# Keep-Passion/ImageStitch

Measured on AMD Instinct MI355X. Metric: image-pairs/sec (2048x2048 grayscale, SURF+BF), higher is better.
Workload: dtype f32

## Files before the change

### imagestitch_amd/csrc/match_kernels.hip

```cpp
#include "common.h"
#include <algorithm>
#include <stdlib.h>
#include <math.h>

typedef float float2v __attribute__((ext_vector_type(2)));
typedef const float __attribute__((address_space(4))) cfloat;
typedef float f16v __attribute__((ext_vector_type(16)));

#define SLOAD16(dst, ptr) asm volatile("s_load_dwordx16 %0, %1, 0x0" : "=s"(dst) : "s"(ptr))
#define SLOAD16_BEFORE(dst, ptr, live) asm volatile("s_load_dwordx16 %0, %2, 0x0" : "=s"(dst), "+s"(live) : "s"(ptr))
#define SWAIT(dst) asm volatile("s_waitcnt lgkmcnt(0)" : "+s"(dst))
#define SWAIT2(d0, d1) asm volatile("s_waitcnt lgkmcnt(0)" : "+s"(d0), "+s"(d1))
#define BF_CHUNK(buf, base)                                                                    \
    _Pragma("unroll") for (int d = 0; d < 16; d += 4) {                                        \
        float2v e0 = qv[base + d + 0] - buf[d + 0];                                            \
        float2v e1 = qv[base + d + 1] - buf[d + 1];                                            \
        float2v e2 = qv[base + d + 2] - buf[d + 2];                                            \
        float2v e3 = qv[base + d + 3] - buf[d + 3];                                            \
        acc += e0 * e0 + e1 * e1 + e2 * e2 + e3 * e3;                                          \
    }

__device__ __forceinline__ void knn_update(float dsq, int j, float &b1, float &b2, int &i1, float &b1sq, float &b2sq)
{
    if (dsq < b2sq) {
// ... 204 lines not shown
                S.m1 = fminf(S.m1, v);
                S.thr = S.m2 + BFM_MARGIN;
            }
        }
    }
}

__global__ __launch_bounds__(256, 2) void k_bf_mfma_d64(const MatchDev *jobs)
{
    const MatchDev &J = jobs[blockIdx.z];
    const int nq = __builtin_amdgcn_readfirstlane(*J.nq_ptr), nt = __builtin_amdgcn_readfirstlane(*J.nt_ptr);
    const int lane = threadIdx.x & 63, wave = threadIdx.x >> 6;
    const int q0 = (blockIdx.x * 4 + wave) * 64;
    if (q0 >= nq) return;
    const int nsplit = gridDim.y, sp = blockIdx.y;
    const int ntiles = (nt + 31) >> 5;
    const int tchunk = (ntiles + nsplit - 1) / nsplit;
    const int tile0 = sp * tchunk, tile1 = min(ntiles, tile0 + tchunk);
    const int col = lane & 31, half = lane >> 5;
    float bq0[32], bq1[32];
    {
        const float4 *p0 = reinterpret_cast<const float4 *>(J.q + (size_t)min(q0 + col, nq - 1) * 64 + 32 * half);
        const float4 *p1 = reinterpret_cast<const float4 *>(J.q + (size_t)min(q0 + 32 + col, nq - 1) * 64 + 32 * half);
#pragma unroll
        for (int s4 = 0; s4 < 8; s4++) {
            const float4 u = p0[s4], v = p1[s4];
            bq0[4 * s4 + 0] = -2.f * u.x; bq0[4 * s4 + 1] = -2.f * u.y; bq0[4 * s4 + 2] = -2.f * u.z; bq0[4 * s4 + 3] = -2.f * u.w;
            bq1[4 * s4 + 0] = -2.f * v.x; bq1[4 * s4 + 1] = -2.f * v.y; bq1[4 * s4 + 2] = -2.f * v.z; bq1[4 * s4 + 3] = -2.f * v.w;
        }
    }
    const float baug = half == 0 ? 1.f : 0.f;
    const bool va = q0 + col < nq, vb = q0 + 32 + col < nq;
    BfmState Sa = {INFINITY, INFINITY, INFINITY, 0}, Sb = {INFINITY, INFINITY, INFINITY, 0};
    const size_t pitch = (size_t)J.capq;
    const int lst = sp * 2 + half;
    uint2 *lista = J.c_ent + (size_t)lst * BFM_CAPL * pitch + (q0 + col), *listb = lista + 32;
    const float *T = J.t;
    for (int pass = 0; pass < 2; pass++) {
        const int tend = pass == 0 ? min(tile0 + 1, tile1) : tile1;
        float4 an[8];
        if (tile0 < tend) {
            const float4 *pn = reinterpret_cast<const float4 *>(T + (size_t)min(tile0 * 32 + col, nt - 1) * 64 + 32 * half);
#pragma unroll
            for (int s4 = 0; s4 < 8; s4++) an[s4] = pn[s4];
        }
        for (int tl = tile0; tl < tend; tl++) {
            float a[32];
#pragma unroll
            for (int s4 = 0; s4 < 8; s4++) { a[4 * s4] = an[s4].x; a[4 * s4 + 1] = an[s4].y; a[4 * s4 + 2] = an[s4].z; a[4 * s4 + 3] = an[s4].w; }
            if (tl + 1 < tend) {
                const float4 *pn = reinterpret_cast<const float4 *>(T + (size_t)min((tl + 1) * 32 + col, nt - 1) * 64 + 32 * half);
#pragma unroll
                for (int s4 = 0; s4 < 8; s4++) an[s4] = pn[s4];
            }
            float part = 0.f;
#pragma unroll
            for (int s = 0; s < 32; s++) part += a[s] * a[s];
            const float tnorm = part + __shfl_xor(part, 32, 64);
            const float aaug = half == 0 ? (tl * 32 + col < nt ? tnorm : BFM_FAR) : 0.f;
            f16v acc0 = {0, 0, 0, 0, 0, 0, 0, 0, 0, 0, 0, 0, 0, 0, 0, 0}, acc1 = acc0;
#pragma unroll
            for (int s = 0; s < 32; s++) {
                acc0 = __builtin_amdgcn_mfma_f32_32x32x2f32(a[s], bq0[s], acc0, 0, 0, 0);
                acc1 = __builtin_amdgcn_mfma_f32_32x32x2f32(a[s], bq1[s], acc1, 0, 0, 0);
            }
            acc0 = __builtin_amdgcn_mfma_f32_32x32x2f32(aaug, baug, acc0, 0, 0, 0);
            acc1 = __builtin_amdgcn_mfma_f32_32x32x2f32(aaug, baug, acc1, 0, 0, 0);
            if (pass == 0) {
                bfm_warm(acc0, Sa); bfm_warm(acc1, Sb);
            } else {
                const int row0 = tl * 32 + 4 * half;
                bfm_scan(acc0, Sa, row0, lista, pitch, tl != tile0); bfm_scan(acc1, Sb, row0, listb, pitch, tl != tile0);
            }
        }
        if (pass == 0) {
            Sa.thr = va ? Sa.m2 + BFM_MARGIN : -INFINITY;
            Sb.thr = vb ? Sb.m2 + BFM_MARGIN : -INFINITY;
        }
    }
    if (va) J.c_cnt[(size_t)lst * pitch + q0 + col] = Sa.cnt;
    if (vb) J.c_cnt[(size_t)lst * pitch + q0 + 32 + col] = Sb.cnt;
}

#define BF16_ROW 144
#define BF16_FRAGS 9
typedef short s8v __attribute__((ext_vector_type(8)));

__device__ __forceinline__ unsigned short bf16_rne(float x)
{
    unsigned u = __float_as_uint(x);
    u += 0x7fffu + ((u >> 16) & 1u);
    return (unsigned short)(u >> 16);
}
__device__ __forceinline__ float bf16_to_f32(unsigned short h) { return __uint_as_float((unsigned)h << 16); }

__global__ __launch_bounds__(256) void k_bf_split16(const MatchDev *jobs, float scale_q)
{
    const MatchDev &J = jobs[blockIdx.z];
    const bool is_t = blockIdx.y == 1;
    const int n = is_t ? *J.nt_ptr : *J.nq_ptr;
    const int row = blockIdx.x * 128 + (threadIdx.x >> 1), half = threadIdx.x & 1;
    if (row >= n) return;
    const float *src = (is_t ? J.t : J.q) + (size_t)row * 64 + 32 * half;
    const float sc = is_t ? 1.f : scale_q;
    float part = 0.f;
    s8v hi[4], lo[4];
#pragma unroll
    for (int d = 0; d < 32; d++) {
        const float x = src[d];
        part += x * x;
        const float xs = x * sc;
        const unsigned short h = bf16_rne(xs);
        hi[d >> 3][d & 7] = (short)h;
        lo[d >> 3][d & 7] = (short)bf16_rne(xs - bf16_to_f32(h));
    }
    const float tot = part + __shfl_xor(part, 1, 64);
    s8v ns = {0, 0, 0, 0, 0, 0, 0, 0};
    if (half == 0) {
        unsigned short a = 0x3f80, b = 0x3f80;
        if (is_t) { a = bf16_rne(tot); b = bf16_rne(tot - bf16_to_f32(a)); }
        ns[0] = (short)a; ns[1] = (short)b;
    }
    if (is_t) {
        s8v *dst = reinterpret_cast<s8v *>(J.t16) + (size_t)(row >> 5) * (BF16_FRAGS * 64) + (row & 31) + 32 * half;
#pragma unroll
        for (int s4 = 0; s4 < 4; s4++) { dst[s4 * 64] = hi[s4]; dst[(4 + s4) * 64] = lo[s4]; }
        dst[8 * 64] = ns;
    } else {
        s8v *dst = reinterpret_cast<s8v *>(J.q16 + (size_t)row * BF16_ROW + 64 * half);
#pragma unroll
        for (int s4 = 0; s4 < 4; s4++) { dst[s4] = hi[s4]; dst[4 + s4] = lo[s4]; }
        if (half == 0) *reinterpret_cast<s8v *>(J.q16 + (size_t)row * BF16_ROW + 128) = ns;
    }
}

#ifndef VFSMS_BF_SKIP
#define VFSMS_BF_SKIP 0
#endif
#ifndef BFM_GLDS
#define BFM_GLDS 1
#endif
#define BFM_HI_ERR 1.6e-2f
#define GASM __attribute__((address_space(1)))
typedef GASM const s8v *g_cs8v;
typedef float f2v __attribute__((ext_vector_type(2)));

#ifdef VFSMS_DESC_TIMING
__device__ unsigned long long g_bf_cycles[2][8];
extern "C" int vfsms_debug_bf_cycles(unsigned long long *out) { return hipMemcpyFromSymbol(out, HIP_SYMBOL(g_bf_cycles), sizeof(unsigned long long) * 16) == hipSuccess ? 0 : -3; }
#define BT_DECL unsigned long long _bt[5] = {0, 0, 0, 0, 0}, _bt0 = clock64(), _btl = _bt0
#define BT_MARK(ph) do { const unsigned long long _n = clock64(); _bt[ph] += _n - _btl; _btl = _n; } while (0)
#define BT_FLUSH(pass) do { if ((threadIdx.x & 63) == 0) { for (int _q = 0; _q < 5; _q++) atomicAdd(&g_bf_cycles[pass][_q], _bt[_q]); \
        atomicAdd(&g_bf_cycles[pass][5], clock64() - _bt0); atomicAdd(&g_bf_cycles[pass][6], 1ull); } } while (0)
#else
#define BT_DECL do {} while (0)
#define BT_MARK(ph) do {} while (0)
#define BT_FLUSH(pass) do {} while (0)
#endif
template <int PASS>
__global__ __launch_bounds__(256, 3) void k_bf_mfma16_d64(const MatchDev *jobs, int qblocks, int nsplit, int njobs)
{
    unsigned unit, qb;
    xcd_roi_map(blockIdx.x, (unsigned)qblocks, (unsigned)(nsplit * njobs), unit, qb);
    const int sp = (int)(unit % (unsigned)nsplit);
    const MatchDev &J = jobs[unit / (unsigned)nsplit];
    const int nq = __builtin_amdgcn_readfirstlane(*J.nq_ptr), nt = __builtin_amdgcn_readfirstlane(*J.nt_ptr);
    const int lane = threadIdx.x & 63, wave = threadIdx.x >> 6;
    if ((int)qb * 256 >= nq) return;
    BT_DECL;
    const int q0 = ((int)qb * 4 + wave) * 64;
    const bool live = q0 < nq;
    const int ntiles = (nt + 31) >> 5;
    const int tchunk = (ntiles + nsplit - 1) / nsplit;
    const int tile0 = sp * tchunk, tile1 = min(ntiles, tile0 + tchunk);
    const int col = lane & 31, half = lane >> 5;
    const s8v zero = {0, 0, 0, 0, 0, 0, 0, 0};
    s8v bh0[4], bl0[4], bh1[4], bl1[4], bn0, bn1;
    {
        g_cs8v p0 = (g_cs8v)(J.q16 + (size_t)min(q0 + col, nq - 1) * BF16_ROW + 64 * half);
        g_cs8v p1 = (g_cs8v)(J.q16 + (size_t)min(q0 + 32 + col, nq - 1) * BF16_ROW + 64 * half);
#pragma unroll
        for (int s4 = 0; s4 < 4; s4++) {
            bh0[s4] = p0[s4]; bh1[s4] = p1[s4];
            if (PASS == 1) { bl0[s4] = p0[4 + s4]; bl1[s4] = p1[4 + s4]; } else { bl0[s4] = zero; bl1[s4] = zero; }
        }
        bn0 = half == 0 ? *(g_cs8v)(J.q16 + (size_t)min(q0 + col, nq - 1) * BF16_ROW + 128) : zero;
        bn1 = half == 0 ? *(g_cs8v)(J.q16 + (size_t)min(q0 + 32 + col, nq - 1) * BF16_ROW + 128) : zero;
    }
    constexpr int NFR = PASS == 0 ? 5 : BF16_FRAGS;
    constexpr int BFM_UNIT = 2;
    __shared__ s8v stage[2][BFM_UNIT][NFR * 64];
    g_cs8v T = (g_cs8v)J.t16;
    const int tid = threadIdx.x; (void)tid;
#if BFM_GLDS
    constexpr int NSET = 1;
    const int wv_u = __builtin_amdgcn_readfirstlane(wave);
    auto glds16 = [&](g_cs8v src, const s8v *dst) {
        __builtin_amdgcn_global_load_lds((const __attribute__((address_space(1))) void *)src, (__attribute__((address_space(3))) void *)dst, 16, 0, 0);
    };
    auto fetch = [&](int unit, int b) {
#pragma unroll
        for (int u = 0; u < BFM_UNIT; u++) {
            const int tl = min(tile0 + unit * BFM_UNIT + u, tile1 - 1);
            g_cs8v pn = T + (size_t)tl * (BF16_FRAGS * 64);
            glds16(pn + 64 * wv_u + lane, &stage[b][u][64 * wv_u]);
            if (PASS == 1) {
                glds16(pn + 256 + 64 * wv_u + lane, &stage[b][u][256 + 64 * wv_u]);
                if (wv_u == 0) glds16(pn + 512 + lane, &stage[b][u][PASS == 1 ? 512 : 0]);
            } else if (wv_u == 0) glds16(pn + 512 + lane, &stage[b][u][256]);
        }
    };
    const int nunits = (tile1 - tile0 + BFM_UNIT - 1) / BFM_UNIT;
    if (nunits > 0) fetch(0, 0);
#else
    constexpr int NSET = PASS == 0 ? 2 : 1;
    s8v g0[NSET][BFM_UNIT], g1[NSET][BFM_UNIT], g2[NSET][BFM_UNIT];
#pragma unroll
    for (int e = 0; e < NSET; e++)
#pragma unroll
        for (int u = 0; u < BFM_UNIT; u++) { g0[e][u] = zero; g1[e][u] = zero; g2[e][u] = zero; }
    const int nunits = (tile1 - tile0 + BFM_UNIT - 1) / BFM_UNIT;
    auto fetch = [&](int unit, int e) {
#pragma unroll
        for (int u = 0; u < BFM_UNIT; u++) {
            const int tl = min(tile0 + unit * BFM_UNIT + u, tile1 - 1);
            g_cs8v pn = T + (size_t)tl * (BF16_FRAGS * 64);
            g0[e][u] = pn[tid];
            if (PASS == 1) { g1[e][u] = pn[256 + tid]; g2[e][u] = pn[512 + (tid & 63)]; }
            else g1[e][u] = pn[512 + (tid & 63)];
        }
    };
    auto put = [&](int b, int e) {
#pragma unroll
        for (int u = 0; u < BFM_UNIT; u++) {
            stage[b][u][tid] = g0[e][u];
            if (PASS == 1) { stage[b][u][256 + tid] = g1[e][u]; if (tid < 64) stage[b][u][512 + tid] = g2[e][u]; }
            else if (tid < 64) stage[b][u][256 + tid] = g1[e][u];
        }
    };
    if (nunits > 0) fetch(0, 0);
#endif
#pragma unroll
    for (int s4 = 0; s4 < 4; s4++) {
        asm volatile("" : "+v"(bh0[s4]), "+v"(bh1[s4]));
        if (PASS == 1) asm volatile("" : "+v"(bl0[s4]), "+v"(bl1[s4]));
    }
    asm volatile("" : "+v"(bn0), "+v"(bn1));
    const bool va = q0 + col < nq, vb = q0 + 32 + col < nq;
    const size_t pitch = (size_t)J.capq;
    const int lst = sp * 2 + half, nl = 2 * nsplit;
    float m1a = INFINITY, m2a = INFINITY, m1b = INFINITY, m2b = INFINITY;
    float thra = -INFINITY, thrb = -INFINITY;
    int cnta = 0, cntb = 0;
    if (PASS == 1) {
        GASM const f2v *B = (GASM const f2v *)J.c_m12;
        float a1 = INFINITY, a2 = INFINITY, b1 = INFINITY, b2 = INFINITY;
        for (int L0 = 0; L0 < nl; L0 += 4) {
            f2v ua[4], ub[4];
#pragma unroll
            for (int k = 0; k < 4; k++) {
                const size_t row = (size_t)min(L0 + k, nl - 1) * pitch;
                ua[k] = B[row + min(q0 + col, nq - 1)]; ub[k] = B[row + min(q0 + 32 + col, nq - 1)];
            }
#pragma unroll
            for (int k = 0; k < 4; k++) {
                if (L0 + k >= nl) break;
                a2 = fminf(fminf(a2, ua[k].y), fmaxf(a1, ua[k].x)); a1 = fminf(a1, ua[k].x);
                b2 = fminf(fminf(b2, ub[k].y), fmaxf(b1, ub[k].x)); b1 = fminf(b1, ub[k].x);
            }
        }
        if (va) thra = a2 + (BFM_HI_ERR + BFM_MARGIN);
        if (vb) thrb = b2 + (BFM_HI_ERR + BFM_MARGIN);
    }
    GASM unsigned long long *lista = (GASM unsigned long long *)J.c_ent + (size_t)lst * BFM_CAPL * pitch + (q0 + col), *listb = lista + 32;
#if !BFM_GLDS
    if (nunits > 0) {
        put(0, 0);
#pragma unroll
        for (int k = 1; k <= NSET; k++) fetch(min(k, nunits - 1), k % NSET);
    }
#endif
    BT_MARK(0);
    for (int unit0 = 0; unit0 < nunits; unit0 += NSET) {
#pragma unroll
      for (int v = 0; v < NSET; v++) {
        const int unit = unit0 + v;
        if (unit >= nunits) break;
        const int b = unit & 1;
#if BFM_GLDS
        asm volatile("s_waitcnt vmcnt(0)" ::: "memory");
#endif
        __syncthreads();
        BT_MARK(1);
#if BFM_GLDS
        if (unit + 1 < nunits) fetch(unit + 1, b ^ 1);
#else
        if (unit + 1 < nunits) put(b ^ 1, (v + 1) % NSET);
        fetch(min(unit + 1 + NSET, nunits - 1), (v + 1) % NSET);
#endif
        BT_MARK(2);
        if (!live) continue;
#pragma unroll
        for (int u = 0; u < BFM_UNIT; u++) {
            const int tl = tile0 + unit * BFM_UNIT + u;
            if (tl >= tile1) break;
            const s8v *st = stage[b][u];
            f16v acc0 = {0, 0, 0, 0, 0, 0, 0, 0, 0, 0, 0, 0, 0, 0, 0, 0}, acc1 = acc0;
#if VFSMS_BF_SKIP
            if (PASS == 1) {
                s8v ah[4];
#pragma unroll
                for (int s = 0; s < 4; s++) {
                    ah[s] = st[s * 64 + lane];
                    acc0 = __builtin_amdgcn_mfma_f32_32x32x16_bf16(ah[s], bh0[s], acc0, 0, 0, 0);
                    acc1 = __builtin_amdgcn_mfma_f32_32x32x16_bf16(ah[s], bh1[s], acc1, 0, 0, 0);
                }
                const s8v na = st[(NFR - 1) * 64 + lane];
                acc0 = __builtin_amdgcn_mfma_f32_32x32x16_bf16(na, bn0, acc0, 0, 0, 0);
                acc1 = __builtin_amdgcn_mfma_f32_32x32x16_bf16(na, bn1, acc1, 0, 0, 0);
                float pa = fminf(fminf(acc0[0], acc0[1]), fminf(acc0[2], acc0[3])), pb = fminf(fminf(acc1[0], acc1[1]), fminf(acc1[2], acc1[3]));
#pragma unroll
                for (int i = 4; i < 16; i += 3) {
                    pa = fminf(pa, fminf(acc0[i], fminf(acc0[i + 1], acc0[i + 2])));
                    pb = fminf(pb, fminf(acc1[i], fminf(acc1[i + 1], acc1[i + 2])));
                }
                const bool need0 = __any(pa <= thra + (BFM_HI_ERR + BFM_MARGIN)), need1 = __any(pb <= thrb + (BFM_HI_ERR + BFM_MARGIN));
                if (!need0 && !need1) continue;
                if (need0) {
#pragma unroll
                    for (int s = 0; s < 4; s++) {
                        const s8v al = st[(4 + s) * 64 + lane];
                        acc0 = __builtin_amdgcn_mfma_f32_32x32x16_bf16(ah[s], bl0[s], acc0, 0, 0, 0);
                        acc0 = __builtin_amdgcn_mfma_f32_32x32x16_bf16(al, bh0[s], acc0, 0, 0, 0);
                    }
                } else {
#pragma unroll
                    for (int i = 0; i < 16; i++) acc0[i] = BFM_FAR;
                }
                if (need1) {
#pragma unroll
                    for (int s = 0; s < 4; s++) {
                        const s8v al = st[(4 + s) * 64 + lane];
                        acc1 = __builtin_amdgcn_mfma_f32_32x32x16_bf16(ah[s], bl1[s], acc1, 0, 0, 0);
                        acc1 = __builtin_amdgcn_mfma_f32_32x32x16_bf16(al, bh1[s], acc1, 0, 0, 0);
                    }
                } else {
#pragma unroll
                    for (int i = 0; i < 16; i++) acc1[i] = BFM_FAR;
                }
            } else
#endif
            {
#pragma unroll
            for (int s = 0; s < 4; s++) {
                const s8v ah = st[s * 64 + lane];
                acc0 = __builtin_amdgcn_mfma_f32_32x32x16_bf16(ah, bh0[s], acc0, 0, 0, 0);
                acc1 = __builtin_amdgcn_mfma_f32_32x32x16_bf16(ah, bh1[s], acc1, 0, 0, 0);
                if (PASS == 1) {
                    const s8v al = st[(4 + s) * 64 + lane];
                    acc0 = __builtin_amdgcn_mfma_f32_32x32x16_bf16(ah, bl0[s], acc0, 0, 0, 0);
                    acc1 = __builtin_amdgcn_mfma_f32_32x32x16_bf16(ah, bl1[s], acc1, 0, 0, 0);
                    acc0 = __builtin_amdgcn_mfma_f32_32x32x16_bf16(al, bh0[s], acc0, 0, 0, 0);
                    acc1 = __builtin_amdgcn_mfma_f32_32x32x16_bf16(al, bh1[s], acc1, 0, 0, 0);
                }
            }
            const s8v na = st[(NFR - 1) * 64 + lane];
            acc0 = __builtin_amdgcn_mfma_f32_32x32x16_bf16(na, bn0, acc0, 0, 0, 0);
            acc1 = __builtin_amdgcn_mfma_f32_32x32x16_bf16(na, bn1, acc1, 0, 0, 0);
            }
            if (tl * 32 + 31 >= nt) {
#pragma unroll
                for (int i = 0; i < 16; i++) {
                    const bool past = tl * 32 + 4 * half + (i & 3) + 8 * (i >> 2) >= nt;
                    acc0[i] = past ? BFM_FAR : acc0[i]; acc1[i] = past ? BFM_FAR : acc1[i];
                }
            }
            if (PASS == 0) {
                float ta = fminf(fminf(acc0[0], acc0[1]), fminf(acc0[2], acc0[3])), tb = fminf(fminf(acc1[0], acc1[1]), fminf(acc1[2], acc1[3]));
#pragma unroll
                for (int i = 4; i < 16; i += 3) {
                    ta = fminf(ta, fminf(acc0[i], fminf(acc0[i + 1], acc0[i + 2])));
                    tb = fminf(tb, fminf(acc1[i], fminf(acc1[i + 1], acc1[i + 2])));
                }
                m2a = fminf(m2a, fmaxf(m1a, ta)); m1a = fminf(m1a, ta);
                m2b = fminf(m2b, fmaxf(m1b, tb)); m1b = fminf(m1b, tb);
            } else {
                const int row0 = tl * 32 + 4 * half;
#pragma unroll
                for (int h = 0; h < 2; h++) {
                    const f16v &acc = h == 0 ? acc0 : acc1;
                    const float thr = h == 0 ? thra : thrb;
                    float gm[5];
                    gm[0] = fminf(fminf(acc[0], acc[1]), fminf(acc[2], acc[3]));
#pragma unroll
                    for (int g = 1; g < 5; g++) gm[g] = fminf(acc[3 * g + 1], fminf(acc[3 * g + 2], acc[3 * g + 3]));
                    const float mn = fminf(fminf(gm[0], fminf(gm[1], gm[2])), fminf(gm[3], gm[4]));
                    const bool some = __any(mn <= thr);
                    BT_MARK(3);
                    if (some) {
                        GASM unsigned long long *list = h == 0 ? lista : listb;
                        int cnt = h == 0 ? cnta : cntb;
#pragma unroll
                        for (int g = 0; g < 5; g++) {
                            if (!__any(gm[g] <= thr)) continue;
#pragma unroll
                            for (int i = (g == 0 ? 0 : 3 * g + 1); i < (g == 0 ? 4 : 3 * g + 4); i++) {
                                const float v = acc[i];
                                if (v <= thr && v < 1e29f) {
                                    if (cnt < BFM_CAPL) list[cnt * pitch] = (unsigned long long)__float_as_uint(v) | ((unsigned long long)(unsigned)(row0 + (i & 3) + 8 * (i >> 2)) << 32);
                                    cnt++;
                                }
                            }
                        }
                        if (h == 0) cnta = cnt; else cntb = cnt;
                        BT_MARK(4);
                    }
                }
            }
            if (PASS == 0) BT_MARK(3);
        }
      }
    }
    BT_FLUSH(PASS);
    if (PASS == 0) {
        GASM f2v *B = (GASM f2v *)J.c_m12;
        if (va) B[(size_t)lst * pitch + q0 + col] = f2v{m1a, m2a};
        if (vb) B[(size_t)lst * pitch + q0 + 32 + col] = f2v{m1b, m2b};
    } else {
        if (va) J.c_cnt[(size_t)lst * pitch + q0 + col] = cnta;
        if (vb) J.c_cnt[(size_t)lst * pitch + q0 + 32 + col] = cntb;
    }
}

#define BFV_HITS 12
#ifdef VFSMS_DESC_TIMING
__device__ unsigned g_bfv_stats[4];
extern "C" int vfsms_debug_bfv_stats(unsigned *out) { return hipMemcpyFromSymbol(out, HIP_SYMBOL(g_bfv_stats), sizeof(unsigned) * 4) == hipSuccess ? 0 : -3; }
#define BFV_STAT(i, v) atomicAdd(&g_bfv_stats[i], (unsigned)(v))
#else
#define BFV_STAT(i, v) do {} while (0)
#endif
__device__ __forceinline__ void bfv_exact(const float *__restrict__ Qr, const float *__restrict__ T, int idx, float &B1, float &B2, int &I1)
{
    const float4 *tr = reinterpret_cast<const float4 *>(T + (size_t)idx * 64);
    const float4 *qr = reinterpret_cast<const float4 *>(Qr);
    float acc = 0.f;
#pragma unroll
    for (int d4 = 0; d4 < 16; d4++) {
        const float4 tv = tr[d4], qv = qr[d4];
        const float e0 = qv.x - tv.x, e1 = qv.y - tv.y, e2 = qv.z - tv.z, e3 = qv.w - tv.w;
        acc += e0 * e0 + e1 * e1 + e2 * e2 + e3 * e3;
    }
    const float d = sqrtf(acc);
    if (d < B1 || (d == B1 && idx < I1)) { B2 = B1; B1 = d; I1 = idx; }
    else B2 = fminf(B2, d);
}

__global__ __launch_bounds__(256) void k_bf_verify_d64(const MatchDev *jobs, int cns)
{
    const MatchDev &J = jobs[blockIdx.y];
    const int nq = __builtin_amdgcn_readfirstlane(*J.nq_ptr), nt = __builtin_amdgcn_readfirstlane(*J.nt_ptr);
    if ((int)(blockIdx.x * 256) >= nq) return;
    const int q = blockIdx.x * 256 + threadIdx.x;
    const bool live = q < nq;
    const int nl = 2 * cns;
    const size_t pitch = (size_t)J.capq;
    __shared__ int hits[BFV_HITS][256];
    float s1 = INFINITY, s2 = INFINITY; bool overflow = false;
    if (live)
        for (int L = 0; L < nl; L++) {
            const int c = J.c_cnt[(size_t)L * pitch + q];
            overflow = overflow || c > BFM_CAPL;
            const uint2 *e = J.c_ent + (size_t)L * BFM_CAPL * pitch + q;
            for (int k = 0; k < min(c, BFM_CAPL); k++) {
                const float v = __uint_as_float(e[k * pitch].x);
                s2 = fminf(s2, fmaxf(s1, v));
                s1 = fminf(s1, v);
            }
        }
    const float cut = s2 + BFM_MARGIN;
    if (live) { BFV_STAT(0, 1); BFV_STAT(1, overflow ? 1 : 0); }
    const float *Qr = J.q + (size_t)min(q, nq - 1) * 64;
    float B1 = INFINITY, B2 = INFINITY; int I1 = -1;
    int nh = 0;
    if (live && !overflow)
        for (int L = 0; L < nl; L++) {
            const int c = min(J.c_cnt[(size_t)L * pitch + q], BFM_CAPL);
            const uint2 *e = J.c_ent + (size_t)L * BFM_CAPL * pitch + q;
            for (int k = 0; k < c; k++) {
                const uint2 ev = e[k * pitch];
                if (__uint_as_float(ev.x) <= cut) {
                    if (nh < BFV_HITS) hits[nh++][threadIdx.x] = (int)ev.y;
                    else bfv_exact(Qr, J.t, (int)ev.y, B1, B2, I1);
                }
            }
        }
    if (live) BFV_STAT(3, nh);
    int maxh = nh;
#pragma unroll
    for (int d = 32; d >= 1; d >>= 1) maxh = max(maxh, __shfl_xor(maxh, d, 64));
    for (int k = 0; k < maxh; k++)
        if (k < nh) bfv_exact(Qr, J.t, hits[k][threadIdx.x], B1, B2, I1);
    {
        const int lane = threadIdx.x & 63;
        unsigned long long om = __ballot(live && overflow);
        while (om) {
            const int src = __ffsll((long long)om) - 1;
            om &= om - 1;
            const int qo = __shfl(q, src, 64);
            const float *Qo = J.q + (size_t)qo * 64;
            float b1 = INFINITY, b2 = INFINITY; int i1 = -1;
            for (int j = lane; j < nt; j += 64) bfv_exact(Qo, J.t, j, b1, b2, i1);
#pragma unroll
            for (int d = 32; d >= 1; d >>= 1) {
                const float ob1 = __shfl_xor(b1, d, 64), ob2 = __shfl_xor(b2, d, 64);
                const int oi1 = __shfl_xor(i1, d, 64);
                if (ob1 < b1 || (ob1 == b1 && oi1 >= 0 && (i1 < 0 || oi1 < i1))) { b2 = fminf(b1, ob2); b1 = ob1; i1 = oi1; }
                else b2 = fminf(b2, ob1);
            }
            if (lane == src) { B1 = b1; B2 = b2; I1 = i1; }
        }
    }
    if (live) { J.p_d1[q] = B1; J.p_d2[q] = B2; J.p_i1[q] = I1; }
}

__global__ __launch_bounds__(256) void k_merge_ratio(const MatchDev *jobs, double ratio, int do_ratio)
{
    const MatchDev &J = jobs[blockIdx.y];
    const int nq = __builtin_amdgcn_readfirstlane(*J.nq_ptr), nt = __builtin_amdgcn_readfirstlane(*J.nt_ptr);
    const int q = blockIdx.x * 256 + threadIdx.x;
    if (q >= nq) return;
    float B1 = INFINITY, B2 = INFINITY; int I1 = -1;
    for (int s = 0; s < J.nsplit; s++) {
        const size_t o = (size_t)s * J.capq + q;
        float d = J.p_d1[o]; int i = J.p_i1[o];
        if (i >= 0) {
            if (d < B1) { B2 = B1; B1 = d; I1 = i; } else if (d < B2) { B2 = d; }
            float e = J.p_d2[o];
            if (e < B1) { B2 = B1; B1 = e; } else if (e < B2) { B2 = e; }
        }
    }
    J.d1[q] = B1; J.d2[q] = B2; J.i1[q] = I1;
    if (!do_ratio) return;
    int ok = (I1 >= 0) && (nt >= 2) && ((double)B1 < (double)B2 * ratio);
    int vote = 0;
    if (ok && J.kq) {
        float ay = J.kq[2 * q + 1], ax = J.kq[2 * q];
        float by = J.kt[2 * I1 + 1], bx = J.kt[2 * I1];
        int dx = (int)(ay - by), dy = (int)(ax - bx);
        vote = !(dx == 0 && dy == 0);
        J.votes[2 * (size_t)(J.capq + q)] = dx;
        J.votes[2 * (size_t)(J.capq + q) + 1] = dy;
    }
    J.match_flag[q] = ok | (vote << 1);
}

__device__ __forceinline__ int wave_incl_scan_i(int v)
{
    const int lane = threadIdx.x & 63;
#pragma unroll
    for (int d = 1; d < 64; d <<= 1) {
        int n = __shfl_up(v, d, 64);
        if (lane >= d) v += n;
// ... 167 lines not shown
    b += 3 * al(sizeof(float) * capq) + 2 * al(sizeof(int) * capq);
    b += al(sizeof(int32_t) * 2 * capq) + al(sizeof(int32_t) * 4 * capq) + al(64) + al(64) + al(64);
    return b + 4096;
}

int match_carve(vfsms_ctx *ctx, MatchDev *m, int capq, int dim, int nsplit)
{
    m->capq = capq; m->dim = dim; m->nsplit = nsplit;
    m->p_d1 = (float *)ctx_arena_alloc(ctx, sizeof(float) * (size_t)capq * nsplit);
    m->p_d2 = (float *)ctx_arena_alloc(ctx, sizeof(float) * (size_t)capq * nsplit);
    m->p_i1 = (int *)ctx_arena_alloc(ctx, sizeof(int) * (size_t)capq * nsplit);
    m->d1 = (float *)ctx_arena_alloc(ctx, sizeof(float) * capq);
    m->d2 = (float *)ctx_arena_alloc(ctx, sizeof(float) * capq);
    m->i1 = (int *)ctx_arena_alloc(ctx, sizeof(int) * capq);
    m->match_flag = (int *)ctx_arena_alloc(ctx, sizeof(int) * capq);
    m->match_pos = (int *)ctx_arena_alloc(ctx, sizeof(int) * capq);
    m->pairs = (int32_t *)ctx_arena_alloc(ctx, sizeof(int32_t) * 2 * capq);
    m->votes = (int32_t *)ctx_arena_alloc(ctx, sizeof(int32_t) * 4 * capq);
    m->mcount = (int *)ctx_arena_alloc(ctx, 64);
    m->vsum = (unsigned long long *)ctx_arena_alloc(ctx, 64);
    m->result = (int32_t *)ctx_arena_alloc(ctx, 64);
    if (!m->result) { vfsms_set_error("arena exhausted while carving a match job"); return VFSMS_ERR_CAPACITY; }
    return VFSMS_OK;
}

__global__ __launch_bounds__(256) void k_max_norm2_d64(const float *a, int n, unsigned *out)
{
    const int row = blockIdx.x * 4 + (threadIdx.x >> 6), lane = threadIdx.x & 63;
    if (row >= n) return;
    const float v = a[(size_t)row * 64 + lane];
    float s = v * v;
#pragma unroll
    for (int d = 32; d >= 1; d >>= 1) s += __shfl_xor(s, d, 64);
    if (lane == 0) atomicMax(out, __float_as_uint(s == s ? s : INFINITY));
}

int launch_max_norm2_d64(vfsms_ctx *ctx, const float *a, int n, unsigned *d_out)
{
    if (n > 0) hipLaunchKernelGGL(k_max_norm2_d64, dim3((n + 3) / 4), dim3(256), 0, ctx->stream, a, n, d_out);
    HIP_TRY(hipGetLastError());
    return VFSMS_OK;
}

size_t match_filter_bytes(int capq, int capt, int cns)
{
    return al(sizeof(uint2) * (size_t)capq * cns * 2 * BFM_CAPL) + al(sizeof(int) * (size_t)capq * cns * 2) +
           al(sizeof(unsigned short) * BF16_ROW * (size_t)capq) + al(sizeof(unsigned short) * BF16_ROW * ((size_t)capt + 32)) +
           al(sizeof(float2) * (size_t)capq * cns * 2) + 1024;
}

int match_filter_carve(vfsms_ctx *ctx, MatchDev *m, int capq, int capt, int cns)
{
    m->c_ent = (uint2 *)ctx_arena_alloc(ctx, sizeof(uint2) * (size_t)capq * cns * 2 * BFM_CAPL);
    m->c_cnt = (int *)ctx_arena_alloc(ctx, sizeof(int) * (size_t)capq * cns * 2);
    m->q16 = (unsigned short *)ctx_arena_alloc(ctx, sizeof(unsigned short) * BF16_ROW * (size_t)capq);
    m->t16 = (unsigned short *)ctx_arena_alloc(ctx, sizeof(unsigned short) * BF16_ROW * ((size_t)capt + 32));
    m->c_m12 = (float2 *)ctx_arena_alloc(ctx, sizeof(float2) * (size_t)capq * cns * 2);
    if (!m->c_cnt || !m->t16 || !m->c_m12) { vfsms_set_error("arena exhausted while carving a match filter"); return VFSMS_ERR_CAPACITY; }
    return VFSMS_OK;
}

static bool bf_f32_filter()
{
    static const bool v = getenv("VFSMS_BF_F32FILTER") && atoi(getenv("VFSMS_BF_F32FILTER")) != 0;
    return v;
}

int launch_bf_l2_filtered(vfsms_ctx *ctx, const MatchDev *d_jobs, int njobs, int capq, int capt, int cns)
{
    if (njobs <= 0 || capq <= 0) return VFSMS_OK;
    {
        ProfScope ps(ctx, "bf_mfma");
        if (bf_f32_filter())
            hipLaunchKernelGGL(k_bf_mfma_d64, dim3((capq + 255) / 256, cns, njobs), dim3(256), 0, ctx->stream, d_jobs);
        else {
            hipLaunchKernelGGL(k_bf_split16, dim3((std::max(capq, capt) + 127) / 128, 2, njobs), dim3(256), 0, ctx->stream, d_jobs, -2.f);
            const int qblocks = (capq + 255) / 256;
            hipLaunchKernelGGL(k_bf_mfma16_d64<0>, dim3((unsigned)qblocks * cns * njobs), dim3(256), 0, ctx->stream, d_jobs, qblocks, cns, njobs);
            hipLaunchKernelGGL(k_bf_mfma16_d64<1>, dim3((unsigned)qblocks * cns * njobs), dim3(256), 0, ctx->stream, d_jobs, qblocks, cns, njobs);
        }
    }
    {
        ProfScope ps(ctx, "bf_verify");
        hipLaunchKernelGGL(k_bf_verify_d64, dim3((capq + 255) / 256, njobs), dim3(256), 0, ctx->stream, d_jobs, cns);
    }
    HIP_TRY(hipGetLastError());
    return VFSMS_OK;
}

int launch_bf_l2(vfsms_ctx *ctx, const MatchDev *d_jobs, int njobs, int capq, int nsplit, int dim)
{
    if (njobs <= 0 || capq <= 0) return VFSMS_OK;
    ProfScope ps(ctx, "bf_l2");
    if (dim == 64) {
        hipLaunchKernelGGL(k_bf_l2_d64, dim3((capq + 511) / 512, nsplit, njobs), dim3(256), 0, ctx->stream, d_jobs);
    } else if (dim == 128) {
        hipLaunchKernelGGL(k_bf_l2_gen<128>, dim3((capq + 255) / 256, nsplit, njobs), dim3(256), 0, ctx->stream, d_jobs);
    } else if (dim == 32) {
        hipLaunchKernelGGL(k_bf_l2_gen<32>, dim3((capq + 255) / 256, nsplit, njobs), dim3(256), 0, ctx->stream, d_jobs);
    } else {
        vfsms_set_error("bf_l2: descriptor dim %d unsupported (64, 128, 32)", dim);
        return VFSMS_ERR_UNSUPPORTED;
    }
    HIP_TRY(hipGetLastError());
    return VFSMS_OK;
}

int launch_pack_i8_d128(vfsms_ctx *ctx, const PackJob *d_jobs, int njobs, int max_rows)
{
    if (njobs <= 0 || max_rows <= 0) return VFSMS_OK;
    ProfScope ps(ctx, "pack_i8");
    hipLaunchKernelGGL(k_pack_i8_d128, dim3((max_rows + 63) / 64, njobs), dim3(256), 0, ctx->stream, d_jobs);
    HIP_TRY(hipGetLastError());
    return VFSMS_OK;
}

int launch_bf_i8_d128(vfsms_ctx *ctx, const MatchDev *d_jobs, int njobs, int capq, int nsplit)
{
    if (njobs <= 0 || capq <= 0) return VFSMS_OK;
    ProfScope ps(ctx, "bf_i8");
    hipLaunchKernelGGL(k_bf_i8_d128, dim3((capq + 255) / 256, nsplit, njobs), dim3(256), 0, ctx->stream, d_jobs);
    HIP_TRY(hipGetLastError());
    return VFSMS_OK;
}

static int launch_vote_tail(vfsms_ctx *ctx, const MatchDev *d_jobs, int njobs, int capq, int estimator, int tol, int offset_evaluate)
{
    if (estimator == VFSMS_OFFSET_CONSENSUS) {
        hipLaunchKernelGGL(k_match_scan, dim3(njobs), dim3(1024), 0, ctx->stream, d_jobs);
        HIP_TRY(hipGetLastError());
        return launch_consensus(ctx, d_jobs, njobs, capq, tol, offset_evaluate);
    }
    hipLaunchKernelGGL(k_scan_mode, dim3(njobs), dim3(1024), 0, ctx->stream, d_jobs, offset_evaluate);
    HIP_TRY(hipGetLastError());
    return VFSMS_OK;
}

static int verify_tail(vfsms_ctx *ctx, const MatchDev *d_jobs, int njobs)
{
    if (ctx->offset_verifier != VFSMS_VERIFY_NCC) return VFSMS_OK;
    return launch_verify(ctx, d_jobs, njobs, ctx->verify_threshold, ctx->verify_min_pixels);
}

int launch_ratio_mode(vfsms_ctx *ctx, const MatchDev *d_jobs, int njobs, int capq, double ratio, int offset_evaluate)
{
    if (njobs <= 0) return VFSMS_OK;
    {
        ProfScope ps(ctx, "vote");
        hipLaunchKernelGGL(k_merge_ratio, dim3((capq + 255) / 256, njobs), dim3(256), 0, ctx->stream, d_jobs, ratio, 1);
        TRY(launch_vote_tail(ctx, d_jobs, njobs, capq, ctx->offset_estimator, ctx->offset_tol, offset_evaluate));
    }
    return verify_tail(ctx, d_jobs, njobs);
}

int launch_ratio_only(vfsms_ctx *ctx, const MatchDev *d_jobs, int njobs, int capq, double ratio)
{
    hipLaunchKernelGGL(k_merge_ratio, dim3((capq + 255) / 256, njobs), dim3(256), 0, ctx->stream, d_jobs, ratio, 1);
    hipLaunchKernelGGL(k_match_scan, dim3(njobs), dim3(1024), 0, ctx->stream, d_jobs);
    HIP_TRY(hipGetLastError());
    return VFSMS_OK;
}

int launch_merge_only(vfsms_ctx *ctx, const MatchDev *d_jobs, int njobs, int capq)
{
    hipLaunchKernelGGL(k_merge_ratio, dim3((capq + 255) / 256, njobs), dim3(256), 0, ctx->stream, d_jobs, 0.0, 0);
    HIP_TRY(hipGetLastError());
    return VFSMS_OK;
// ... 31 lines not shown
```

Baseline: 2337.

## Replace split-bf16 hi/lo distance filter with single fp16 MFMA pass

```diff
diff --git a/imagestitch_amd/csrc/match_kernels.hip b/imagestitch_amd/csrc/match_kernels.hip
--- a/imagestitch_amd/csrc/match_kernels.hip
+++ b/imagestitch_amd/csrc/match_kernels.hip
@@ -310,17 +310,10 @@
     if (vb) J.c_cnt[(size_t)lst * pitch + q0 + 32 + col] = Sb.cnt;
 }
 
-#define BF16_ROW 144
-#define BF16_FRAGS 9
-typedef short s8v __attribute__((ext_vector_type(8)));
-
-__device__ __forceinline__ unsigned short bf16_rne(float x)
-{
-    unsigned u = __float_as_uint(x);
-    u += 0x7fffu + ((u >> 16) & 1u);
-    return (unsigned short)(u >> 16);
-}
-__device__ __forceinline__ float bf16_to_f32(unsigned short h) { return __uint_as_float((unsigned)h << 16); }
+#define BF16_ROW 80
+#define BF16_FRAGS 5
+#define BFM_F16_ERR 2.0e-3f
+typedef _Float16 h8v __attribute__((ext_vector_type(8)));
 
 __global__ __launch_bounds__(256) void k_bf_split16(const MatchDev *jobs, float scale_q)
 {
@@ -332,45 +325,39 @@
     const float *src = (is_t ? J.t : J.q) + (size_t)row * 64 + 32 * half;
     const float sc = is_t ? 1.f : scale_q;
     float part = 0.f;
-    s8v hi[4], lo[4];
+    h8v el[4];
 #pragma unroll
     for (int d = 0; d < 32; d++) {
         const float x = src[d];
         part += x * x;
-        const float xs = x * sc;
-        const unsigned short h = bf16_rne(xs);
-        hi[d >> 3][d & 7] = (short)h;
-        lo[d >> 3][d & 7] = (short)bf16_rne(xs - bf16_to_f32(h));
+        el[d >> 3][d & 7] = (_Float16)(x * sc);
     }
     const float tot = part + __shfl_xor(part, 1, 64);
-    s8v ns = {0, 0, 0, 0, 0, 0, 0, 0};
+    h8v ns = {0, 0, 0, 0, 0, 0, 0, 0};
     if (half == 0) {
-        unsigned short a = 0x3f80, b = 0x3f80;
-        if (is_t) { a = bf16_rne(tot); b = bf16_rne(tot - bf16_to_f32(a)); }
-        ns[0] = (short)a; ns[1] = (short)b;
+        _Float16 a = (_Float16)1.f, b = (_Float16)1.f;
+        if (is_t) { a = (_Float16)tot; b = (_Float16)(tot - (float)a); }
+        ns[0] = a; ns[1] = b;
     }
     if (is_t) {
-        s8v *dst = reinterpret_cast<s8v *>(J.t16) + (size_t)(row >> 5) * (BF16_FRAGS * 64) + (row & 31) + 32 * half;
-#pragma unroll
-        for (int s4 = 0; s4 < 4; s4++) { dst[s4 * 64] = hi[s4]; dst[(4 + s4) * 64] = lo[s4]; }
-        dst[8 * 64] = ns;
+        h8v *dst = reinterpret_cast<h8v *>(J.t16) + (size_t)(row >> 5) * (BF16_FRAGS * 64) + (row & 31) + 32 * half;
+#pragma unroll
+        for (int s4 = 0; s4 < 4; s4++) dst[s4 * 64] = el[s4];
+        dst[4 * 64] = ns;
     } else {
-        s8v *dst = reinterpret_cast<s8v *>(J.q16 + (size_t)row * BF16_ROW + 64 * half);
-#pragma unroll
-        for (int s4 = 0; s4 < 4; s4++) { dst[s4] = hi[s4]; dst[4 + s4] = lo[s4]; }
-        if (half == 0) *reinterpret_cast<s8v *>(J.q16 + (size_t)row * BF16_ROW + 128) = ns;
-    }
-}
-
-#ifndef VFSMS_BF_SKIP
-#define VFSMS_BF_SKIP 0
-#endif
+        h8v *dst = reinterpret_cast<h8v *>(J.q16 + (size_t)row * BF16_ROW + 32 * half);
+#pragma unroll
+        for (int s4 = 0; s4 < 4; s4++) dst[s4] = el[s4];
+        if (half == 0) *reinterpret_cast<h8v *>(J.q16 + (size_t)row * BF16_ROW + 64) = ns;
+    }
+}
+
 #ifndef BFM_GLDS
 #define BFM_GLDS 1
 #endif
-#define BFM_HI_ERR 1.6e-2f
+#define BFM_WINDOW (2.f * BFM_F16_ERR + BFM_MARGIN)
 #define GASM __attribute__((address_space(1)))
-typedef GASM const s8v *g_cs8v;
+typedef GASM const h8v *g_cs8v;
 typedef float f2v __attribute__((ext_vector_type(2)));
 
 #ifdef VFSMS_DESC_TIMING
@@ -402,28 +389,25 @@
     const int tchunk = (ntiles + nsplit - 1) / nsplit;
     const int tile0 = sp * tchunk, tile1 = min(ntiles, tile0 + tchunk);
     const int col = lane & 31, half = lane >> 5;
-    const s8v zero = {0, 0, 0, 0, 0, 0, 0, 0};
-    s8v bh0[4], bl0[4], bh1[4], bl1[4], bn0, bn1;
+    const h8v zero = {0, 0, 0, 0, 0, 0, 0, 0};
+    h8v bh0[4], bh1[4], bn0, bn1;
     {
-        g_cs8v p0 = (g_cs8v)(J.q16 + (size_t)min(q0 + col, nq - 1) * BF16_ROW + 64 * half);
-        g_cs8v p1 = (g_cs8v)(J.q16 + (size_t)min(q0 + 32 + col, nq - 1) * BF16_ROW + 64 * half);
-#pragma unroll
-        for (int s4 = 0; s4 < 4; s4++) {
-            bh0[s4] = p0[s4]; bh1[s4] = p1[s4];
-            if (PASS == 1) { bl0[s4] = p0[4 + s4]; bl1[s4] = p1[4 + s4]; } else { bl0[s4] = zero; bl1[s4] = zero; }
-        }
-        bn0 = half == 0 ? *(g_cs8v)(J.q16 + (size_t)min(q0 + col, nq - 1) * BF16_ROW + 128) : zero;
-        bn1 = half == 0 ? *(g_cs8v)(J.q16 + (size_t)min(q0 + 32 + col, nq - 1) * BF16_ROW + 128) : zero;
-    }
-    constexpr int NFR = PASS == 0 ? 5 : BF16_FRAGS;
+        g_cs8v p0 = (g_cs8v)(J.q16 + (size_t)min(q0 + col, nq - 1) * BF16_ROW + 32 * half);
+        g_cs8v p1 = (g_cs8v)(J.q16 + (size_t)min(q0 + 32 + col, nq - 1) * BF16_ROW + 32 * half);
+#pragma unroll
+        for (int s4 = 0; s4 < 4; s4++) { bh0[s4] = p0[s4]; bh1[s4] = p1[s4]; }
+        bn0 = half == 0 ? *(g_cs8v)(J.q16 + (size_t)min(q0 + col, nq - 1) * BF16_ROW + 64) : zero;
+        bn1 = half == 0 ? *(g_cs8v)(J.q16 + (size_t)min(q0 + 32 + col, nq - 1) * BF16_ROW + 64) : zero;
+    }
+    constexpr int NFR = BF16_FRAGS;
     constexpr int BFM_UNIT = 2;
-    __shared__ s8v stage[2][BFM_UNIT][NFR * 64];
+    __shared__ h8v stage[2][BFM_UNIT][NFR * 64];
     g_cs8v T = (g_cs8v)J.t16;
     const int tid = threadIdx.x; (void)tid;
 #if BFM_GLDS
     constexpr int NSET = 1;
     const int wv_u = __builtin_amdgcn_readfirstlane(wave);
-    auto glds16 = [&](g_cs8v src, const s8v *dst) {
+    auto glds16 = [&](g_cs8v src, const h8v *dst) {
         __builtin_amdgcn_global_load_lds((const __attribute__((address_space(1))) void *)src, (__attribute__((address_space(3))) void *)dst, 16, 0, 0);
     };
     auto fetch = [&](int unit, int b) {
@@ -432,21 +416,18 @@
             const int tl = min(tile0 + unit * BFM_UNIT + u, tile1 - 1);
             g_cs8v pn = T + (size_t)tl * (BF16_FRAGS * 64);
             glds16(pn + 64 * wv_u + lane, &stage[b][u][64 * wv_u]);
-            if (PASS == 1) {
-                glds16(pn + 256 + 64 * wv_u + lane, &stage[b][u][256 + 64 * wv_u]);
-                if (wv_u == 0) glds16(pn + 512 + lane, &stage[b][u][PASS == 1 ? 512 : 0]);
-            } else if (wv_u == 0) glds16(pn + 512 + lane, &stage[b][u][256]);
+            if (wv_u == 0) glds16(pn + 256 + lane, &stage[b][u][256]);
         }
     };
     const int nunits = (tile1 - tile0 + BFM_UNIT - 1) / BFM_UNIT;
     if (nunits > 0) fetch(0, 0);
 #else
     constexpr int NSET = PASS == 0 ? 2 : 1;
-    s8v g0[NSET][BFM_UNIT], g1[NSET][BFM_UNIT], g2[NSET][BFM_UNIT];
+    h8v g0[NSET][BFM_UNIT], g1[NSET][BFM_UNIT];
 #pragma unroll
     for (int e = 0; e < NSET; e++)
 #pragma unroll
-        for (int u = 0; u < BFM_UNIT; u++) { g0[e][u] = zero; g1[e][u] = zero; g2[e][u] = zero; }
+        for (int u = 0; u < BFM_UNIT; u++) { g0[e][u] = zero; g1[e][u] = zero; }
     const int nunits = (tile1 - tile0 + BFM_UNIT - 1) / BFM_UNIT;
     auto fetch = [&](int unit, int e) {
 #pragma unroll
@@ -454,25 +435,20 @@
             const int tl = min(tile0 + unit * BFM_UNIT + u, tile1 - 1);
             g_cs8v pn = T + (size_t)tl * (BF16_FRAGS * 64);
             g0[e][u] = pn[tid];
-            if (PASS == 1) { g1[e][u] = pn[256 + tid]; g2[e][u] = pn[512 + (tid & 63)]; }
-            else g1[e][u] = pn[512 + (tid & 63)];
+            g1[e][u] = pn[256 + (tid & 63)];
         }
     };
     auto put = [&](int b, int e) {
 #pragma unroll
         for (int u = 0; u < BFM_UNIT; u++) {
             stage[b][u][tid] = g0[e][u];
-            if (PASS == 1) { stage[b][u][256 + tid] = g1[e][u]; if (tid < 64) stage[b][u][512 + tid] = g2[e][u]; }
-            else if (tid < 64) stage[b][u][256 + tid] = g1[e][u];
+            if (tid < 64) stage[b][u][256 + tid] = g1[e][u];
         }
     };
     if (nunits > 0) fetch(0, 0);
 #endif
 #pragma unroll
-    for (int s4 = 0; s4 < 4; s4++) {
-        asm volatile("" : "+v"(bh0[s4]), "+v"(bh1[s4]));
-        if (PASS == 1) asm volatile("" : "+v"(bl0[s4]), "+v"(bl1[s4]));
-    }
+    for (int s4 = 0; s4 < 4; s4++) asm volatile("" : "+v"(bh0[s4]), "+v"(bh1[s4]));
     asm volatile("" : "+v"(bn0), "+v"(bn1));
     const bool va = q0 + col < nq, vb = q0 + 32 + col < nq;
     const size_t pitch = (size_t)J.capq;
@@ -497,8 +473,8 @@
                 b2 = fminf(fminf(b2, ub[k].y), fmaxf(b1, ub[k].x)); b1 = fminf(b1, ub[k].x);
             }
         }
-        if (va) thra = a2 + (BFM_HI_ERR + BFM_MARGIN);
-        if (vb) thrb = b2 + (BFM_HI_ERR + BFM_MARGIN);
+        if (va) thra = a2 + BFM_WINDOW;
+        if (vb) thrb = b2 + BFM_WINDOW;
     }
     GASM unsigned long long *lista = (GASM unsigned long long *)J.c_ent + (size_t)lst * BFM_CAPL * pitch + (q0 + col), *listb = lista + 32;
 #if !BFM_GLDS
@@ -532,70 +508,17 @@
         for (int u = 0; u < BFM_UNIT; u++) {
             const int tl = tile0 + unit * BFM_UNIT + u;
             if (tl >= tile1) break;
-            const s8v *st = stage[b][u];
+            const h8v *st = stage[b][u];
             f16v acc0 = {0, 0, 0, 0, 0, 0, 0, 0, 0, 0, 0, 0, 0, 0, 0, 0}, acc1 = acc0;
-#if VFSMS_BF_SKIP
-            if (PASS == 1) {
-                s8v ah[4];
-#pragma unroll
-                for (int s = 0; s < 4; s++) {
-                    ah[s] = st[s * 64 + lane];
-                    acc0 = __builtin_amdgcn_mfma_f32_32x32x16_bf16(ah[s], bh0[s], acc0, 0, 0, 0);
-                    acc1 = __builtin_amdgcn_mfma_f32_32x32x16_bf16(ah[s], bh1[s], acc1, 0, 0, 0);
-                }
-                const s8v na = st[(NFR - 1) * 64 + lane];
-                acc0 = __builtin_amdgcn_mfma_f32_32x32x16_bf16(na, bn0, acc0, 0, 0, 0);
-                acc1 = __builtin_amdgcn_mfma_f32_32x32x16_bf16(na, bn1, acc1, 0, 0, 0);
-                float pa = fminf(fminf(acc0[0], acc0[1]), fminf(acc0[2], acc0[3])), pb = fminf(fminf(acc1[0], acc1[1]), fminf(acc1[2], acc1[3]));
-#pragma unroll
-                for (int i = 4; i < 16; i += 3) {
-                    pa = fminf(pa, fminf(acc0[i], fminf(acc0[i + 1], acc0[i + 2])));
-                    pb = fminf(pb, fminf(acc1[i], fminf(acc1[i + 1], acc1[i + 2])));
-                }
-                const bool need0 = __any(pa <= thra + (BFM_HI_ERR + BFM_MARGIN)), need1 = __any(pb <= thrb + (BFM_HI_ERR + BFM_MARGIN));
-                if (!need0 && !need1) continue;
-                if (need0) {
-#pragma unroll
-                    for (int s = 0; s < 4; s++) {
-                        const s8v al = st[(4 + s) * 64 + lane];
-                        acc0 = __builtin_amdgcn_mfma_f32_32x32x16_bf16(ah[s], bl0[s], acc0, 0, 0, 0);
-                        acc0 = __builtin_amdgcn_mfma_f32_32x32x16_bf16(al, bh0[s], acc0, 0, 0, 0);
-                    }
-                } else {
-#pragma unroll
-                    for (int i = 0; i < 16; i++) acc0[i] = BFM_FAR;
-                }
-                if (need1) {
-#pragma unroll
-                    for (int s = 0; s < 4; s++) {
-                        const s8v al = st[(4 + s) * 64 + lane];
-                        acc1 = __builtin_amdgcn_mfma_f32_32x32x16_bf16(ah[s], bl1[s], acc1, 0, 0, 0);
-                        acc1 = __builtin_amdgcn_mfma_f32_32x32x16_bf16(al, bh1[s], acc1, 0, 0, 0);
-                    }
-                } else {
-#pragma unroll
-                    for (int i = 0; i < 16; i++) acc1[i] = BFM_FAR;
-                }
-            } else
-#endif
-            {
 #pragma unroll
             for (int s = 0; s < 4; s++) {
-                const s8v ah = st[s * 64 + lane];
-                acc0 = __builtin_amdgcn_mfma_f32_32x32x16_bf16(ah, bh0[s], acc0, 0, 0, 0);
-                acc1 = __builtin_amdgcn_mfma_f32_32x32x16_bf16(ah, bh1[s], acc1, 0, 0, 0);
-                if (PASS == 1) {
-                    const s8v al = st[(4 + s) * 64 + lane];
-                    acc0 = __builtin_amdgcn_mfma_f32_32x32x16_bf16(ah, bl0[s], acc0, 0, 0, 0);
-                    acc1 = __builtin_amdgcn_mfma_f32_32x32x16_bf16(ah, bl1[s], acc1, 0, 0, 0);
-                    acc0 = __builtin_amdgcn_mfma_f32_32x32x16_bf16(al, bh0[s], acc0, 0, 0, 0);
-                    acc1 = __builtin_amdgcn_mfma_f32_32x32x16_bf16(al, bh1[s], acc1, 0, 0, 0);
-                }
-            }
-            const s8v na = st[(NFR - 1) * 64 + lane];
-            acc0 = __builtin_amdgcn_mfma_f32_32x32x16_bf16(na, bn0, acc0, 0, 0, 0);
-            acc1 = __builtin_amdgcn_mfma_f32_32x32x16_bf16(na, bn1, acc1, 0, 0, 0);
-            }
+                const h8v at = st[s * 64 + lane];
+                acc0 = __builtin_amdgcn_mfma_f32_32x32x16_f16(at, bh0[s], acc0, 0, 0, 0);
+                acc1 = __builtin_amdgcn_mfma_f32_32x32x16_f16(at, bh1[s], acc1, 0, 0, 0);
+            }
+            const h8v na = st[(NFR - 1) * 64 + lane];
+            acc0 = __builtin_amdgcn_mfma_f32_32x32x16_f16(na, bn0, acc0, 0, 0, 0);
+            acc1 = __builtin_amdgcn_mfma_f32_32x32x16_f16(na, bn1, acc1, 0, 0, 0);
             if (tl * 32 + 31 >= nt) {
 #pragma unroll
                 for (int i = 0; i < 16; i++) {
@@ -684,7 +607,7 @@
     else B2 = fminf(B2, d);
 }
 
-__global__ __launch_bounds__(256) void k_bf_verify_d64(const MatchDev *jobs, int cns)
+__global__ __launch_bounds__(256) void k_bf_verify_d64(const MatchDev *jobs, int cns, float window)
 {
     const MatchDev &J = jobs[blockIdx.y];
     const int nq = __builtin_amdgcn_readfirstlane(*J.nq_ptr), nt = __builtin_amdgcn_readfirstlane(*J.nt_ptr);
@@ -699,6 +622,7 @@
         for (int L = 0; L < nl; L++) {
             const int c = J.c_cnt[(size_t)L * pitch + q];
             overflow = overflow || c > BFM_CAPL;
+            BFV_STAT(2, min(c, BFM_CAPL));
             const uint2 *e = J.c_ent + (size_t)L * BFM_CAPL * pitch + q;
             for (int k = 0; k < min(c, BFM_CAPL); k++) {
                 const float v = __uint_as_float(e[k * pitch].x);
@@ -706,7 +630,7 @@
                 s1 = fminf(s1, v);
             }
         }
-    const float cut = s2 + BFM_MARGIN;
+    const float cut = s2 + window;
     if (live) { BFV_STAT(0, 1); BFV_STAT(1, overflow ? 1 : 0); }
     const float *Qr = J.q + (size_t)min(q, nq - 1) * 64;
     float B1 = INFINITY, B2 = INFINITY; int I1 = -1;
@@ -1040,7 +964,7 @@
     }
     {
         ProfScope ps(ctx, "bf_verify");
-        hipLaunchKernelGGL(k_bf_verify_d64, dim3((capq + 255) / 256, njobs), dim3(256), 0, ctx->stream, d_jobs, cns);
+        hipLaunchKernelGGL(k_bf_verify_d64, dim3((capq + 255) / 256, njobs), dim3(256), 0, ctx->stream, d_jobs, cns, bf_f32_filter() ? BFM_MARGIN : BFM_WINDOW);
     }
     HIP_TRY(hipGetLastError());
     return VFSMS_OK;
```

After: 2442 (median of 6 runs). +4.5%, better.
